# roclark/torchsr

Measured on AMD Instinct MI355X. Metric: 96x96 HR crops/sec (SRGAN GAN train step), higher is better.
Workload: dtype f32; 1 GPU; SRGAN full GAN step (Generator + Discriminator + VGG19 perceptual loss), 96x96 HR crops, batch 16 per GPU, fp32; per_gpu_batch=16, global_batch=16, crop=96, parallelism=dp1, hip_graph=True, vgg19_weights=seeded-random, plan_cus=256

## Files before the change

torchsr_amd/csrc/convpack.hip:

```cpp
#include "conv_host.h"

namespace {

__global__ void pack_fwd_kernel(const float* __restrict__ w, float* __restrict__ p, int Cout, int Cin, int KH, int KW,
                                int Ck, int K, int Kp, int Cnp, int shuffle_cps) {
  const int64_t idx = (int64_t)blockIdx.x * blockDim.x + threadIdx.x;
  if (idx >= (int64_t)Cnp * Kp) return;
  const int np = (int)(idx / Kp), k = (int)(idx - (int64_t)np * Kp);
  float v = 0.f;
  if (np < Cout && k < K) {
    const int tap = k / Ck, ci = k - tap * Ck;
    if (ci < Cin) {
      int co = np;
      if (shuffle_cps) { const int ij = np / shuffle_cps, cc = np - ij * shuffle_cps; co = cc * 4 + ij; }
      const int kh = tap / KW, kw = tap - kh * KW;
      v = w[(((size_t)co * Cin + ci) * KH + kh) * KW + kw];
    }
  }
  p[idx] = v;
}

__global__ void pack_bwd_kernel(const float* __restrict__ w, float* __restrict__ p, int Cout, int Cin, int KH, int KW,
                                int stride, int pad, int ph, int pw, int dminh, int dminw, int ntw, int Ck, int K,
                                int Kp, int Cnp, int shuffle_cps) {
  const int64_t idx = (int64_t)blockIdx.x * blockDim.x + threadIdx.x;
  if (idx >= (int64_t)Cnp * Kp) return;
  const int ci = (int)(idx / Kp), k = (int)(idx - (int64_t)ci * Kp);
  float v = 0.f;
  if (ci < Cin && k < K) {
    const int tap = k / Ck, c = k - tap * Ck;
    if (c < Cout) {
      const int th = tap / ntw, tw = tap - th * ntw;
      const int kh = ph + pad - stride * (dminh + th), kw = pw + pad - stride * (dminw + tw);
      int co = c;
      if (shuffle_cps) { const int ij = c / shuffle_cps, cc = c - ij * shuffle_cps; co = cc * 4 + ij; }
      v = w[(((size_t)co * Cin + ci) * KH + kh) * KW + kw];
    }
  }
  p[idx] = v;
}

struct PackSeg { float* dst; int rows, K, Kp, Ck, bwd, ph, pw, dminh, dminw, ntw; };
struct PackArgs {
  const float* w;
  int Cout, Cin, KH, KW, stride, pad, cps, nseg;
  PackSeg seg[17];
};
__global__ void pack_all_kernel(const PackArgs a) {
  const PackSeg sg = a.seg[blockIdx.y];
  const int64_t idx = (int64_t)blockIdx.x * blockDim.x + threadIdx.x;
  if (idx >= (int64_t)sg.rows * sg.Kp) return;
  const int row = (int)(idx / sg.Kp), k = (int)(idx - (int64_t)row * sg.Kp);
  float v = 0.f;
  if (k < sg.K) {
    const int tap = k / sg.Ck, c = k - tap * sg.Ck;
    if (!sg.bwd) {
      if (row < a.Cout && c < a.Cin) {
        int co = row;
        if (a.cps) { const int ij = row / a.cps, cc = row - ij * a.cps; co = cc * 4 + ij; }
        const int kh = tap / a.KW, kw = tap - kh * a.KW;
        v = a.w[(((size_t)co * a.Cin + c) * a.KH + kh) * a.KW + kw];
      }
    } else {
      if (row < a.Cin && c < a.Cout) {
        const int th = tap / sg.ntw, tw = tap - th * sg.ntw;
        const int kh = sg.ph + a.pad - a.stride * (sg.dminh + th), kw = sg.pw + a.pad - a.stride * (sg.dminw + tw);
        int co = c;
        if (a.cps) { const int ij = c / a.cps, cc = c - ij * a.cps; co = cc * 4 + ij; }
        v = a.w[(((size_t)co * a.Cin + row) * a.KH + kh) * a.KW + kw];
      }
    }
  }
  sg.dst[idx] = v;
}

}

extern "C" int srx_conv2d_pack(const srx_conv2d_t* d, const float* w, float* wpk_fwd, float* wpk_bwd, void* stream) {
  if (int rc = check_desc(d)) return rc;
  SRX_REQUIRE(w && wpk_fwd, "conv2d_pack: null pointer");
  hipStream_t st = srx_stream(stream);
  const Geo g = fwd_geo(d);
  PackArgs pa{};
  pa.w = w; pa.Cout = d->Cout; pa.Cin = d->Cin; pa.KH = d->KH; pa.KW = d->KW; pa.stride = d->stride; pa.pad = d->pad;
  pa.cps = g.cps;
  int64_t maxn = 0;
  if (srx_thin_fwd_applicable(d)) {
    if (int rc = srx_thin_pack(d, w, wpk_fwd, 0, st)) return rc;
  } else {
    PackSeg& sg = pa.seg[pa.nseg++];
    sg = PackSeg{wpk_fwd, g.Cnp, g.K, g.Kp, g.Ck, 0, 0, 0, 0, 0, 1};
    maxn = (int64_t)g.Cnp * g.Kp;
  }
  if (wpk_bwd && srx_thin_dgrad_applicable(d)) {
    if (int rc = srx_thin_pack(d, w, wpk_bwd, 1, st)) return rc;
  } else if (wpk_bwd) {
    SRX_REQUIRE(d->stride <= 4, "conv2d_pack: stride > 4 unsupported for the data gradient");
    BwdClass cls[16];
    size_t total;
    const int nc = bwd_classes(d, cls, total);
    const int Ck = bwd_ck(d);
    const int Cnp = pad_rows(d->Cin);
    for (int i = 0; i < nc; ++i) {
      const BwdClass& c = cls[i];
      PackSeg& sg = pa.seg[pa.nseg++];
      sg = PackSeg{wpk_bwd + c.woff, Cnp, c.K, c.Kp, Ck, 1, c.ph, c.pw, c.dminh, c.dminw, c.ntw > 0 ? c.ntw : 1};
      if ((int64_t)Cnp * c.Kp > maxn) maxn = (int64_t)Cnp * c.Kp;
    }
  }
  if (pa.nseg > 0) {
    hipLaunchKernelGGL(pack_all_kernel, dim3((unsigned)srx_cdiv(maxn, 256), pa.nseg), dim3(256), 0, st, pa);
    SRX_CHECK_LAUNCH("pack_all_kernel");
  }
  return SRX_OK;
}

struct PackRec {
  float* dst; const float* w;
  long long n_elems;
  int kind;
  int rows, K, Kp, Ck, ph, pw, dminh, dminw, ntw;
  int Cout, Cin, KH, KW, stride, pad, cps, pad_;
};

__global__ void pack_table_kernel(const PackRec* __restrict__ table) {
  const PackRec r = table[blockIdx.y];
  const int64_t idx = (int64_t)blockIdx.x * blockDim.x + threadIdx.x;
  if (idx >= r.n_elems) return;
  float v = 0.f;
  if (r.kind >= 4) {
    srx_wino_pack_one(r.w, r.dst, r.Cout, r.Cin, r.kind == 5 ? 1 : (r.kind == 6 ? 2 : 0), idx);
    return;
  }
  if (r.kind >= 2) {
    const int taps = r.KH * r.KW;
    const int ch = (int)(idx & 63), tap = (int)((idx >> 6) % taps), c = (int)(idx / (64 * taps));
    const int Cthin = r.kind == 2 ? r.Cout : r.Cin;
    if (c < Cthin) {
      const int kh = tap / r.KW, kw = tap - kh * r.KW;
      v = r.kind == 2 ? r.w[(((size_t)c * 64 + ch) * r.KH + kh) * r.KW + kw]
                      : r.w[(((size_t)ch * Cthin + c) * r.KH + (r.KH - 1 - kh)) * r.KW + (r.KW - 1 - kw)];
    }
    r.dst[idx] = v;
    return;
  }
  const int taps = r.K / r.Ck;
  const int64_t nmain = (int64_t)r.rows * r.Ck;
  if (idx >= nmain) {
    const int padk = r.Kp - r.K;
    const int64_t j = idx - nmain;
    if (padk > 0 && j < (int64_t)r.rows * padk) {
      const int row = (int)(j / padk);
      r.dst[(size_t)row * r.Kp + r.K + (int)(j - (int64_t)row * padk)] = 0.f;
    }
    return;
  }
  const int row = (int)(idx / r.Ck), c = (int)(idx - (int64_t)row * r.Ck);
  float* d = r.dst + (size_t)row * r.Kp + c;
  const bool live = r.kind == 0 ? (row < r.Cout && c < r.Cin) : (row < r.Cin && c < r.Cout);
  int co = r.kind == 0 ? row : c;
  if (r.cps) { const int ij = co / r.cps, cc = co - ij * r.cps; co = cc * 4 + ij; }
  const float* src = r.w + ((size_t)co * r.Cin + (r.kind == 0 ? c : row)) * (r.KH * r.KW);
  for (int t0 = 0; t0 < taps; t0 += 9) {
    float v[9];
#pragma unroll
    for (int u = 0; u < 9; ++u) {
      const int tap = min(t0 + u, taps - 1);
      int off = tap;
      if (r.kind == 1) {
        const int th = tap / r.ntw, tw = tap - th * r.ntw;
        off = (r.ph + r.pad - r.stride * (r.dminh + th)) * r.KW + (r.pw + r.pad - r.stride * (r.dminw + tw));
      }
      v[u] = live ? src[off] : 0.f;
    }
#pragma unroll
    for (int u = 0; u < 9; ++u)
      if (t0 + u < taps) d[(size_t)(t0 + u) * r.Ck] = v[u];
  }
}

extern "C" size_t srx_pack_table_bytes(int n_layers) { return (size_t)n_layers * 17 * sizeof(PackRec); }

extern "C" int srx_pack_table_build(const srx_conv2d_t* descs, int n, const float* const* w, float* const* wpk_fwd,
                                    float* const* wpk_bwd, void* host_table, int* nrec_out, long long* max_elems_out) {
  SRX_REQUIRE(descs && w && wpk_fwd && wpk_bwd && host_table && nrec_out && max_elems_out && n > 0,
              "pack_table_build: bad argument");
  PackRec* out = static_cast<PackRec*>(host_table);
  int nrec = 0;
  long long maxn = 0;
  for (int i = 0; i < n; ++i) {
    const srx_conv2d_t* d = descs + i;
    if (int rc = check_desc(d)) return rc;
    SRX_REQUIRE(w[i] && wpk_fwd[i], "pack_table_build: null pointer in layer %d", i);
    const Geo g = fwd_geo(d);
    PackRec base{};
    base.w = w[i];
    base.Cout = d->Cout; base.Cin = d->Cin; base.KH = d->KH; base.KW = d->KW; base.stride = d->stride; base.pad = d->pad;
    base.cps = g.cps;
    auto emit = [&](PackRec r) {
      if (r.n_elems > maxn) maxn = r.n_elems;
      out[nrec++] = r;
    };
    if (srx_thin_fwd_applicable(d)) {
      PackRec r = base; r.kind = 2; r.dst = wpk_fwd[i]; r.n_elems = 4LL * d->KH * d->KW * 64; emit(r);
    } else {
      PackRec r = base; r.kind = 0; r.dst = wpk_fwd[i]; r.rows = g.Cnp; r.K = g.K; r.Kp = g.Kp; r.Ck = g.Ck; r.ntw = 1;
      r.n_elems = (long long)g.Cnp * (g.Ck + g.Kp - g.K); emit(r);
    }
    if (!wpk_bwd[i]) continue;
    if (srx_thin_dgrad_applicable(d)) {
      PackRec r = base; r.kind = 3; r.dst = wpk_bwd[i]; r.n_elems = 4LL * d->KH * d->KW * 64; emit(r);
      continue;
    }
    SRX_REQUIRE(d->stride <= 4, "pack_table_build: stride > 4 unsupported for the data gradient");
    BwdClass cls[16];
    size_t total;
    const int nc = bwd_classes(d, cls, total);
    const int Cnp = pad_rows(d->Cin);
    for (int c = 0; c < nc; ++c) {
      PackRec r = base; r.kind = 1; r.dst = wpk_bwd[i] + cls[c].woff;
      r.rows = Cnp; r.K = cls[c].K; r.Kp = cls[c].Kp; r.Ck = bwd_ck(d);
      r.ph = cls[c].ph; r.pw = cls[c].pw; r.dminh = cls[c].dminh; r.dminw = cls[c].dminw;
      r.ntw = cls[c].ntw > 0 ? cls[c].ntw : 1;
      r.n_elems = (long long)Cnp * (r.Ck + cls[c].Kp - cls[c].K);
      emit(r);
    }
  }
  *nrec_out = nrec;
  *max_elems_out = maxn;
  return SRX_OK;
}

extern "C" int srx_pack_table_add_wino(void* host_table, int* nrec, long long* max_elems, const srx_conv2d_t* d, const float* w,
                                       float* upk, int transpose) {
  SRX_REQUIRE(host_table && nrec && max_elems && d && w && upk && *nrec >= 0, "pack_table_add_wino: bad argument");
  SRX_REQUIRE(srx_wino_applicable(d) || srx_wino_packed_floats(d) > 0, "pack_table_add_wino: not a Winograd layer");
  PackRec r{};
  SRX_REQUIRE(!(transpose && d->shuffle), "pack_table_add_wino: a PixelShuffle layer has no Winograd data gradient");
  r.dst = upk; r.w = w; r.kind = transpose ? 5 : (d->shuffle ? 6 : 4);
  r.Cout = d->Cout; r.Cin = d->Cin; r.KH = 3; r.KW = 3; r.stride = 1; r.pad = 1;
  r.n_elems = (long long)d->Cout * d->Cin;
  static_cast<PackRec*>(host_table)[(*nrec)++] = r;
  if (r.n_elems > *max_elems) *max_elems = r.n_elems;
  return SRX_OK;
}

extern "C" int srx_pack_table_run(const void* dev_table, int nrec, long long max_elems, void* stream) {
  SRX_REQUIRE(dev_table && nrec > 0 && nrec <= 65535 && max_elems > 0, "pack_table_run: bad argument");
  hipLaunchKernelGGL(pack_table_kernel, dim3((unsigned)srx_cdiv(max_elems, 256), (unsigned)nrec), dim3(256), 0,
                     srx_stream(stream), static_cast<const PackRec*>(dev_table));
  SRX_CHECK_LAUNCH("pack_table_kernel");
  return SRX_OK;
}
```

torchsr_amd/csrc/srx_common.h:

```cpp
#pragma once
#include <hip/hip_runtime.h>
#include <hip/hip_ext.h>
#include <stdint.h>
#include <stddef.h>
#include "../../include/srx.h"

typedef float f32x4 __attribute__((ext_vector_type(4)));
typedef float f32x16 __attribute__((ext_vector_type(16)));

void srx_set_error(const char* fmt, ...);

#define SRX_FAIL(code, ...)      \
  do {                           \
    srx_set_error(__VA_ARGS__);  \
    return (code);               \
  } while (0)

#define SRX_REQUIRE(cond, ...) \
  do {                         \
    if (!(cond)) SRX_FAIL(SRX_E_BADARG, __VA_ARGS__); \
  } while (0)

#define SRX_CHECK_LAUNCH(name)                                                        \
  do {                                                                                \
    hipError_t e__ = hipGetLastError();                                               \
    if (e__ != hipSuccess) SRX_FAIL(SRX_E_HIP, "%s: %s", name, hipGetErrorString(e__)); \
  } while (0)

struct SrxDevSwitches {
  bool no_rt36, no_wgrad_rows, no_bn_bwd_fuse, no_bn_fwd_fuse, no_first3, no_c64, force_plan, no_wgrad_dma, no_wgrad_lin, no_wino, old_wgrad_reduce, wino_no_tail;
  int wgrad_nsplit, wgrad_rows_nsplit, first3_wgs_per_cu, thin_fwd_rows, reserved_cus, c64_ablate, rdb_ablate, wino_zsplit, wino_bn;
  int s2_mode;
  int plan[4];
};
const SrxDevSwitches& srx_dev();
extern "C" int srx_plan_cus(void);

bool srx_prof_on();
bool srx_prof_aux();
bool srx_prof_take(const char* name, double flops, hipEvent_t* e0, hipEvent_t* e1);
#define SRX_LAUNCH_PROF(name, flops, kernel, grid, block, lds, st, ...)                              \
  do {                                                                                               \
    hipEvent_t e0__ = nullptr, e1__ = nullptr;                                                       \
    if (srx_prof_on() && srx_prof_take(name, flops, &e0__, &e1__))                                   \
      hipExtLaunchKernelGGL(kernel, grid, block, (std::uint32_t)(lds), st, e0__, e1__, 0, __VA_ARGS__); \
    else                                                                                             \
      hipLaunchKernelGGL(kernel, grid, block, lds, st, __VA_ARGS__);                                 \
  } while (0)
#define SRX_LAUNCH_PROF_AUX(name, kernel, grid, block, lds, st, ...)                                 \
  do {                                                                                               \
    if (srx_prof_aux()) SRX_LAUNCH_PROF(name, 0.0, kernel, grid, block, lds, st, __VA_ARGS__);       \
    else hipLaunchKernelGGL(kernel, grid, block, lds, st, __VA_ARGS__);                              \
  } while (0)

bool srx_thin_wgrad_applicable(const srx_conv2d_t* d);
size_t srx_thin_wgrad_ws_floats(const srx_conv2d_t* d);
int srx_thin_wgrad(const srx_conv2d_t* d, const float* x, const float* dy, float* dw, int accumulate, float* ws,
                   size_t ws_floats, hipStream_t st);
bool srx_thin_fwd_applicable(const srx_conv2d_t* d);
bool srx_first3_fwd_applicable(const srx_conv2d_t* d);
int srx_first3_fwd(const srx_conv2d_t* d, const float* in, const float* wpk, int Kp, const float* bias, float* out, hipStream_t st, int out_bf16 = 0);
bool srx_thin_dgrad_applicable(const srx_conv2d_t* d);
int srx_thin_pack(const srx_conv2d_t* d, const float* w, float* p, int mode, hipStream_t st);
int srx_thin_fwd(const srx_conv2d_t* d, const float* in, const float* wpk, const float* bias, float* out, int n_out,
                 hipStream_t st, int in_bf16 = 0);

bool srx_rt36_applicable(const srx_conv2d_t* d);
int srx_rt36_rows(const srx_conv2d_t* d);
struct srx_rt36_bn_t { const float* y; const float* mean; const float* invstd; const float* gamma; const float* beta;
                       const float* prelu; float* part; };
struct srx_rt36_bnl_t { const float* mean; const float* invstd; const float* gamma; const float* beta; const float* prelu;
                        const float* res;
                        float* z_out; };
struct srx_rt36_bnb_t { const float* y; const float* mean; const float* invstd; const float* gamma; const float* beta;
                        const float* prelu; const float* sums; float inv_m; float* dy_out; };
int srx_rt36_run(const srx_conv2d_t* d, const float* in, const float* wpk, const float* bias, const float* residual,
                 float* out, float* part, int act, float slope, hipStream_t st, const srx_rt36_bn_t* bn = nullptr,
                 const srx_rt36_bnl_t* bnl = nullptr, const srx_rt36_bnb_t* bnb = nullptr);

static inline hipStream_t srx_stream(void* s) { return (hipStream_t)s; }
static inline int64_t srx_cdiv(int64_t a, int64_t b) { return (a + b - 1) / b; }
static inline int64_t srx_roundup(int64_t a, int64_t b) { return srx_cdiv(a, b) * b; }

__device__ __forceinline__ void srx_divmod(int m, int d, float inv_d, int& q, int& r) {
  q = __float2int_rz(__int2float_rn(m) * inv_d);
  r = m - q * d;
  if (r < 0) { q -= 1; r += d; }
  if (r >= d) { q += 1; r -= d; }
}

__device__ __forceinline__ __amdgpu_buffer_rsrc_t srx_rsrc(const void* p, unsigned bytes) {
  return __builtin_amdgcn_make_buffer_rsrc(const_cast<void*>(p), (short)0, (int)bytes, 0x00020000);
}
__device__ __forceinline__ f32x4 srx_bload(__amdgpu_buffer_rsrc_t r, unsigned voff, unsigned soff) {
  return __builtin_bit_cast(f32x4, __builtin_amdgcn_raw_buffer_load_b128(r, (int)voff, (int)soff, 0));
}
__device__ __forceinline__ int srx_uniform(int v) { return __builtin_amdgcn_readfirstlane(v); }

__device__ __forceinline__ float srx_wave_sum(float v) {
#pragma unroll
  for (int o = 32; o > 0; o >>= 1) v += __shfl_xor(v, o, 64);
  return v;
}

__device__ __forceinline__ void srx_wino_pack_one(const float* __restrict__ w, float* __restrict__ upk, int Cout, int Cin,
                                                  int transpose, int64_t idx) {
  const int R = transpose == 1 ? Cin : Cout, K = transpose == 1 ? Cout : Cin;
  const int r = (int)(idx / K), k = (int)(idx - (int64_t)r * K);
  const int rsrc = transpose == 2 ? (r % (Cout / 4)) * 4 + r / (Cout / 4) : r;
  float g[3][3];
#pragma unroll
  for (int i = 0; i < 3; ++i)
#pragma unroll
    for (int j = 0; j < 3; ++j)
      g[i][j] = transpose == 1 ? w[(((size_t)k * Cin + r) * 3 + (2 - i)) * 3 + (2 - j)] : w[(((size_t)rsrc * Cin + k) * 3 + i) * 3 + j];
  float t[4][3];
#pragma unroll
  for (int j = 0; j < 3; ++j) {
    t[0][j] = g[0][j];
    t[1][j] = 0.5f * (g[0][j] + g[1][j] + g[2][j]);
    t[2][j] = 0.5f * (g[0][j] - g[1][j] + g[2][j]);
    t[3][j] = g[2][j];
  }
  const int nch = K / 32, rt = R / 32;
  const int jg = r >> 5, mrow = r & 31, kc = k / 32, kk = k % 32, quad = kk >> 2, e = kk & 3, s = quad >> 1, hh = quad & 1;
#pragma unroll
  for (int i = 0; i < 4; ++i) {
    const float u[4] = {t[i][0], 0.5f * (t[i][0] + t[i][1] + t[i][2]), 0.5f * (t[i][0] - t[i][1] + t[i][2]), t[i][2]};
#pragma unroll
    for (int j = 0; j < 4; ++j) {
      const int xi = 4 * i + j;
      upk[(((((size_t)xi * rt + jg) * nch + kc) * 4 + s) * 64 + hh * 32 + mrow) * 4 + e] = u[j];
    }
  }
}
```

Before: 2422 crops/s.

## Rework weight pack table kernel into persistent flattened grid with LDS-tiled Winograd packing

Replaces the 2D pack launch (max_elems x nrec blocks, many idle) with a persistent 1D grid sized to CUs times a per-CU block count. Each block walks a contiguous range of flattened work items across records using prefix offsets stored in the table. Winograd weight packing now stages 32x32 filter tiles in shared memory with vectorized loads, so output writes are coalesced. Strided data-gradient packs are merged into one record that reads each weight once and scatters to all parity classes. This cuts wasted blocks and uncoalesced traffic in the per-step weight repack, at the cost of more complex indexing and host-side checks that must match the device class layout.

```diff
diff --git a/torchsr_amd/csrc/convpack.hip b/torchsr_amd/csrc/convpack.hip
--- a/torchsr_amd/csrc/convpack.hip
+++ b/torchsr_amd/csrc/convpack.hip
@@ -1,4 +1,5 @@
 #include "conv_host.h"
+#include <algorithm>
 
 namespace {
 
@@ -120,18 +121,69 @@
   long long n_elems;
   int kind;
   int rows, K, Kp, Ck, ph, pw, dminh, dminw, ntw;
-  int Cout, Cin, KH, KW, stride, pad, cps, pad_;
+  int Cout, Cin, KH, KW, stride, pad, cps;
+  int blk0;
+  int total;
 };
 
-__global__ void pack_table_kernel(const PackRec* __restrict__ table) {
-  const PackRec r = table[blockIdx.y];
-  const int64_t idx = (int64_t)blockIdx.x * blockDim.x + threadIdx.x;
+#ifndef PACK_WGS_PER_CU
+#define PACK_WGS_PER_CU 32
+#endif
+__host__ __device__ inline int rec_items(long long n_elems) { return (int)((n_elems + 255) / 256); }
+
+__host__ __device__ inline int pack_class_taps(int par, int pad, int stride, int Kd, int& dmin) {
+  const int kfirst = (par + pad) % stride;
+  if (kfirst >= Kd) { dmin = 0; return 0; }
+  const int cnt = (Kd - 1 - kfirst) / stride + 1;
+  dmin = (par + pad - kfirst) / stride - (cnt - 1);
+  return cnt;
+}
+
+__device__ __forceinline__ void pack_dgrad_classes(const PackRec& r, int64_t idx) {
+  const int taps = r.KH * r.KW;
+  const int64_t nmain = (int64_t)r.rows * r.Ck;
+  const bool main = idx < nmain;
+  const int64_t j = main ? idx : idx - nmain;
+  const int div = main ? r.Ck : r.K;
+  const int row = (int)(j / div);
+  int c = (int)(j - (int64_t)row * div);
+  float v[9];
+  if (main) {
+    const bool live = row < r.Cin && c < r.Cout;
+    int co = c;
+    if (r.cps) { const int ij = co / r.cps, cc = co - ij * r.cps; co = cc * 4 + ij; }
+    const float* src = r.w + ((size_t)co * r.Cin + row) * taps;
+#pragma unroll
+    for (int u = 0; u < 9; ++u) v[u] = (live && u < taps) ? src[u] : 0.f;
+  }
+  float* cls = r.dst;
+  for (int ph = 0; ph < r.stride; ++ph)
+    for (int pw = 0; pw < r.stride; ++pw) {
+      int dminh, dminw;
+      const int nth = pack_class_taps(ph, r.pad, r.stride, r.KH, dminh), ntw = pack_class_taps(pw, r.pad, r.stride, r.KW, dminw);
+      const int K = nth * ntw * r.Ck, Kp = (int)((max(K, 1) + BK - 1) / BK) * BK;
+      if (main) {
+        float* d = cls + (size_t)row * Kp + c;
+        for (int th = 0; th < nth; ++th)
+          for (int tw = 0; tw < ntw; ++tw) {
+            const int off = (ph + r.pad - r.stride * (dminh + th)) * r.KW + (pw + r.pad - r.stride * (dminw + tw));
+            float x = v[0];
+#pragma unroll
+            for (int u = 1; u < 9; ++u) x = off == u ? v[u] : x;
+            d[(size_t)(th * ntw + tw) * r.Ck] = x;
+          }
+      } else {
+        if (c >= 0 && c < Kp - K) cls[(size_t)row * Kp + K + c] = 0.f;
+        c -= Kp - K;
+      }
+      cls += (size_t)r.rows * Kp;
+    }
+}
+
+__device__ __forceinline__ void pack_item(const PackRec& r, int64_t idx) {
   if (idx >= r.n_elems) return;
+  if (r.kind == 7) { pack_dgrad_classes(r, idx); return; }
   float v = 0.f;
-  if (r.kind >= 4) {
-    srx_wino_pack_one(r.w, r.dst, r.Cout, r.Cin, r.kind == 5 ? 1 : (r.kind == 6 ? 2 : 0), idx);
-    return;
-  }
   if (r.kind >= 2) {
     const int taps = r.KH * r.KW;
     const int ch = (int)(idx & 63), tap = (int)((idx >> 6) % taps), c = (int)(idx / (64 * taps));
@@ -176,6 +228,81 @@
 #pragma unroll
     for (int u = 0; u < 9; ++u)
       if (t0 + u < taps) d[(size_t)(t0 + u) * r.Ck] = v[u];
+  }
+}
+
+constexpr int WTILE_S0 = 76, WTILE_S1 = 292;
+constexpr int WTILE_FLOATS = 32 * WTILE_S0;
+__device__ __forceinline__ void pack_wino_tile(const PackRec& r, int item, float* __restrict__ tile) {
+  const int tr = r.kind == 5 ? 1 : (r.kind == 6 ? 2 : 0);
+  const int R = tr == 1 ? r.Cin : r.Cout, K = tr == 1 ? r.Cout : r.Cin;
+  const int nch = K / 32, rt = R / 32;
+  const int s = item & 3, kc = (item >> 2) % nch, jg = (item >> 2) / nch;
+  const int t = threadIdx.x;
+  __syncthreads();
+  for (int i = t; i < 576; i += 256) {
+    size_t src;
+    int dst;
+    if (tr == 1) {
+      const int kq = i / 72, p = i - kq * 72;
+      src = ((size_t)(kc * 32 + s * 8 + kq) * r.Cin + jg * 32) * 9 + p * 4;
+      dst = kq * WTILE_S1 + p * 4;
+    } else {
+      const int m = i / 18, p = i - m * 18;
+      const int row = jg * 32 + m;
+      const int rsrc = tr == 2 ? (row % (r.Cout / 4)) * 4 + row / (r.Cout / 4) : row;
+      src = ((size_t)rsrc * r.Cin + kc * 32 + s * 8) * 9 + p * 4;
+      dst = m * WTILE_S0 + p * 4;
+    }
+    *reinterpret_cast<f32x4*>(tile + dst) = *reinterpret_cast<const f32x4*>(r.w + src);
+  }
+  __syncthreads();
+  const int e = t & 3, mrow = (t >> 2) & 31, hh = t >> 7, kq = hh * 4 + e;
+  float g[3][3];
+#pragma unroll
+  for (int i = 0; i < 3; ++i)
+#pragma unroll
+    for (int j = 0; j < 3; ++j)
+      g[i][j] = tr == 1 ? tile[kq * WTILE_S1 + mrow * 9 + (2 - i) * 3 + (2 - j)] : tile[mrow * WTILE_S0 + kq * 9 + i * 3 + j];
+  float u[16];
+  srx_wino_transform(g, u);
+  float* d = r.dst + ((size_t)(jg * nch + kc) * 4 + s) * 256 + t;
+  const size_t xstride = (size_t)rt * nch * 1024;
+#pragma unroll
+  for (int xi = 0; xi < 16; ++xi) d[xi * xstride] = u[xi];
+}
+
+__global__ __launch_bounds__(256) void pack_table_kernel(const PackRec* __restrict__ table, int nrec) {
+  __shared__ __attribute__((aligned(16))) float tile[WTILE_FLOATS];
+  __shared__ int s_rec;
+  const int tid = threadIdx.x;
+  const int total = table[0].total;
+  int lo = 0x7fffffff, hi = 0x7fffffff;
+  if (tid < nrec) {
+    lo = table[tid].blk0;
+    if (tid + 1 < nrec) hi = table[tid + 1].blk0;
+  }
+  const int share = (total + (int)gridDim.x - 1) / (int)gridDim.x;
+  const int b0 = blockIdx.x * share, b1 = min(total, b0 + share);
+  if (b0 >= b1) return;
+  if (lo <= b0 && b0 < hi) s_rec = tid;
+  for (int i = tid + 256; i < nrec; i += 256) {
+    const int l = table[i].blk0, h = i + 1 < nrec ? table[i + 1].blk0 : 0x7fffffff;
+    if (l <= b0 && b0 < h) s_rec = i;
+  }
+  __syncthreads();
+  int ri = srx_uniform(s_rec);
+  PackRec r = table[ri];
+  int rend = ri + 1 < nrec ? table[ri + 1].blk0 : total;
+  for (int fb = b0; fb < b1; ++fb) {
+    if (fb >= rend) {
+      ++ri;
+      r = table[ri];
+      rend = ri + 1 < nrec ? table[ri + 1].blk0 : total;
+    }
+    const int item = fb - r.blk0;
+    if (r.kind >= 4 && r.kind <= 6) pack_wino_tile(r, item, tile);
+    else pack_item(r, (int64_t)item * 256 + threadIdx.x);
   }
 }
 
@@ -199,7 +326,9 @@
     base.cps = g.cps;
     auto emit = [&](PackRec r) {
       if (r.n_elems > maxn) maxn = r.n_elems;
+      r.blk0 = nrec ? out[nrec - 1].blk0 + rec_items(out[nrec - 1].n_elems) : 0;
       out[nrec++] = r;
+      out[0].total = r.blk0 + rec_items(r.n_elems);
     };
     if (srx_thin_fwd_applicable(d)) {
       PackRec r = base; r.kind = 2; r.dst = wpk_fwd[i]; r.n_elems = 4LL * d->KH * d->KW * 64; emit(r);
@@ -217,6 +346,25 @@
     size_t total;
     const int nc = bwd_classes(d, cls, total);
     const int Cnp = pad_rows(d->Cin);
+    if (d->stride > 1 && d->KH * d->KW <= 9) {
+      PackRec r = base; r.kind = 7; r.dst = wpk_bwd[i]; r.rows = Cnp; r.Ck = bwd_ck(d);
+      int sumpad = 0;
+      size_t floats = 0;
+      for (int ph = 0, c = 0; ph < d->stride; ++ph)
+        for (int pw = 0; pw < d->stride; ++pw, ++c) {
+          int dminh, dminw;
+          const int nth = pack_class_taps(ph, d->pad, d->stride, d->KH, dminh), ntw = pack_class_taps(pw, d->pad, d->stride, d->KW, dminw);
+          const int K = nth * ntw * r.Ck, Kp = (int)srx_roundup(K > 0 ? K : 1, BK);
+          SRX_REQUIRE(c < nc && cls[c].woff == floats && cls[c].K == K && cls[c].Kp == Kp && cls[c].dminh == dminh && cls[c].dminw == dminw,
+                      "pack_table_build: class %d of layer %d is cut differently on the device", c, i);
+          sumpad += Kp - K;
+          floats += (size_t)Cnp * Kp;
+        }
+      r.K = sumpad;
+      r.n_elems = (long long)Cnp * (r.Ck + sumpad);
+      emit(r);
+      continue;
+    }
     for (int c = 0; c < nc; ++c) {
       PackRec r = base; r.kind = 1; r.dst = wpk_bwd[i] + cls[c].woff;
       r.rows = Cnp; r.K = cls[c].K; r.Kp = cls[c].Kp; r.Ck = bwd_ck(d);
@@ -240,15 +388,19 @@
   r.dst = upk; r.w = w; r.kind = transpose ? 5 : (d->shuffle ? 6 : 4);
   r.Cout = d->Cout; r.Cin = d->Cin; r.KH = 3; r.KW = 3; r.stride = 1; r.pad = 1;
   r.n_elems = (long long)d->Cout * d->Cin;
-  static_cast<PackRec*>(host_table)[(*nrec)++] = r;
+  PackRec* out = static_cast<PackRec*>(host_table);
+  r.blk0 = *nrec ? out[*nrec - 1].blk0 + rec_items(out[*nrec - 1].n_elems) : 0;
+  out[(*nrec)++] = r;
+  out[0].total = r.blk0 + rec_items(r.n_elems);
   if (r.n_elems > *max_elems) *max_elems = r.n_elems;
   return SRX_OK;
 }
 
 extern "C" int srx_pack_table_run(const void* dev_table, int nrec, long long max_elems, void* stream) {
   SRX_REQUIRE(dev_table && nrec > 0 && nrec <= 65535 && max_elems > 0, "pack_table_run: bad argument");
-  hipLaunchKernelGGL(pack_table_kernel, dim3((unsigned)srx_cdiv(max_elems, 256), (unsigned)nrec), dim3(256), 0,
-                     srx_stream(stream), static_cast<const PackRec*>(dev_table));
+  const int64_t grid = std::min<int64_t>((int64_t)srx_plan_cus() * PACK_WGS_PER_CU, srx_cdiv(max_elems, 256) * nrec);
+  hipLaunchKernelGGL(pack_table_kernel, dim3((unsigned)grid), dim3(256), 0, srx_stream(stream),
+                     static_cast<const PackRec*>(dev_table), nrec);
   SRX_CHECK_LAUNCH("pack_table_kernel");
   return SRX_OK;
 }
diff --git a/torchsr_amd/csrc/srx_common.h b/torchsr_amd/csrc/srx_common.h
--- a/torchsr_amd/csrc/srx_common.h
+++ b/torchsr_amd/csrc/srx_common.h
@@ -103,6 +103,24 @@
   return v;
 }
 
+__device__ __forceinline__ void srx_wino_transform(const float (&g)[3][3], float (&u)[16]) {
+  float t[4][3];
+#pragma unroll
+  for (int j = 0; j < 3; ++j) {
+    t[0][j] = g[0][j];
+    t[1][j] = 0.5f * (g[0][j] + g[1][j] + g[2][j]);
+    t[2][j] = 0.5f * (g[0][j] - g[1][j] + g[2][j]);
+    t[3][j] = g[2][j];
+  }
+#pragma unroll
+  for (int i = 0; i < 4; ++i) {
+    u[4 * i + 0] = t[i][0];
+    u[4 * i + 1] = 0.5f * (t[i][0] + t[i][1] + t[i][2]);
+    u[4 * i + 2] = 0.5f * (t[i][0] - t[i][1] + t[i][2]);
+    u[4 * i + 3] = t[i][2];
+  }
+}
+
 __device__ __forceinline__ void srx_wino_pack_one(const float* __restrict__ w, float* __restrict__ upk, int Cout, int Cin,
                                                   int transpose, int64_t idx) {
   const int R = transpose == 1 ? Cin : Cout, K = transpose == 1 ? Cout : Cin;
@@ -114,23 +132,11 @@
 #pragma unroll
     for (int j = 0; j < 3; ++j)
       g[i][j] = transpose == 1 ? w[(((size_t)k * Cin + r) * 3 + (2 - i)) * 3 + (2 - j)] : w[(((size_t)rsrc * Cin + k) * 3 + i) * 3 + j];
-  float t[4][3];
-#pragma unroll
-  for (int j = 0; j < 3; ++j) {
-    t[0][j] = g[0][j];
-    t[1][j] = 0.5f * (g[0][j] + g[1][j] + g[2][j]);
-    t[2][j] = 0.5f * (g[0][j] - g[1][j] + g[2][j]);
-    t[3][j] = g[2][j];
-  }
+  float u[16];
+  srx_wino_transform(g, u);
   const int nch = K / 32, rt = R / 32;
   const int jg = r >> 5, mrow = r & 31, kc = k / 32, kk = k % 32, quad = kk >> 2, e = kk & 3, s = quad >> 1, hh = quad & 1;
 #pragma unroll
-  for (int i = 0; i < 4; ++i) {
-    const float u[4] = {t[i][0], 0.5f * (t[i][0] + t[i][1] + t[i][2]), 0.5f * (t[i][0] - t[i][1] + t[i][2]), t[i][2]};
-#pragma unroll
-    for (int j = 0; j < 4; ++j) {
-      const int xi = 4 * i + j;
-      upk[(((((size_t)xi * rt + jg) * nch + kc) * 4 + s) * 64 + hh * 32 + mrow) * 4 + e] = u[j];
-    }
-  }
+  for (int xi = 0; xi < 16; ++xi)
+    upk[(((((size_t)xi * rt + jg) * nch + kc) * 4 + s) * 64 + hh * 32 + mrow) * 4 + e] = u[xi];
 }
```

Result: no change. 2435 crops/s, median of 6 (+0.5%).
